# aayush9400/3D-Condtional-Stable-Diffusion

Measured on AMD Instinct MI355X. Metric: latent volumes/sec at 32^3x8ch T=1000 DDPM, higher is better.
Workload: dtype f32 (f16 hi+lo x3 MFMA, f32 accumulate)

## Files before the change

### 3d-condtional-stable-diffusion_amd/csrc/dm3d_conv.hip

```cpp
#include <algorithm>
#include <cstdlib>
#include "dm3d_conv_args.h"
#include <math.h>

namespace {

template <int TD, int TH, int TW, int S, int KS, int WM, int WN>
__global__ __launch_bounds__(256, 2) void conv3d_igemm_f32(const ConvArgs p) {
    constexpr int CK = 16, LDV = CK + 4, NT = 64;
    constexpr int TM = TD * TH * TW;
    constexpr int HD = (TD - 1) * S + KS, HH = (TH - 1) * S + KS, HW = (TW - 1) * S + KS;
    constexpr int HVOX = HD * HH * HW;
    constexpr int TAPS = KS * KS * KS;
    constexpr int MR = TM / WM / 32, NR = NT / WN / 32;
    constexpr int NTHR = WM * WN * 64;
    constexpr int NSLOT = (HVOX * 4 + NTHR - 1) / NTHR;
    static_assert(NTHR == 256, "kernel assumes 4 waves");
    static_assert(TM % (WM * 32) == 0 && NT % (WN * 32) == 0, "tile split");

    extern __shared__ __attribute__((aligned(16))) float smem[];
    float* lds_in = smem;
    float* lds_w = smem + HVOX * LDV;

    const int tid = threadIdx.x;
// ... 127 lines not shown
        const int n = n0 + wn * (NT / WN) + nr * 32 + l32;
        const bool n_ok = n < p.cout;
        const int nc = n_ok ? n : p.cout - 1;
        float add = p.bias ? p.bias[nc] : 0.0f;
        if (p.vec) add += p.vec[(size_t)vrow * p.vec_ld + nc];
#pragma unroll
        for (int mr = 0; mr < MR; ++mr) {
            size_t o[16];
            bool ok[16];
            float rv[16];
#pragma unroll
            for (int r = 0; r < 16; ++r) {
                const int row = wm * (TM / WM) + mr * 32 + dm3d_acc_row(r, half);
                const int oz = oz0 + row / (TH * TW), oy = oy0 + (row / TW) % TH, ox = ox0 + row % TW;
                ok[r] = n_ok && oz < p.od && oy < p.oh && ox < p.ow;
                o[r] = ok[r] ? ((((size_t)b * p.fd + oz * p.os + ooz) * p.fh + oy * p.os + ooy) * p.fw + ox * p.os + oox) * p.cout + n : 0;
            }
            if (p.res) {
#pragma unroll
                for (int r = 0; r < 16; ++r) rv[r] = p.res[o[r]];
            }
#pragma unroll
            for (int r = 0; r < 16; ++r) {
                float v = acc[mr][nr][r] + add;
                if (p.relu) v = fmaxf(v, 0.0f);
                if (p.prelu) { const float al = p.prelu[o[r] % sample_elems]; v = v > 0.0f ? v : al * v; }
                if (p.res) v += rv[r];
                if (p.relu_out) v = fmaxf(v, 0.0f);
                if (ok[r]) p.out[o[r]] = v;
            }
        }
    }
}

template <int TD, int TH, int TW, int S, int KS, int WM, int WN>
int launch_conv(ConvArgs& a, hipStream_t st) {
    constexpr int LDV = 20;
    constexpr int HVOX = ((TD - 1) * S + KS) * ((TH - 1) * S + KS) * ((TW - 1) * S + KS);
    constexpr size_t lds = (size_t)(HVOX * LDV + 2 * 64 * LDV) * sizeof(float);
    a.bd = (a.od + TD - 1) / TD;
    a.bh = (a.oh + TH - 1) / TH;
    a.bw = (a.ow + TW - 1) / TW;
    static std::atomic<bool> attr_set[64] = {};
    if (int dev = dm3d_dyn_lds(lds, attr_set, "conv", &conv3d_igemm_f32<TD, TH, TW, S, KS, WM, WN>); dev < 0) return dev;
    dim3 grid((unsigned)(a.batch * a.bd * a.bh * a.bw), (unsigned)(a.coutpad / 64), a.parity ? 8u : 1u);
    hipLaunchKernelGGL((conv3d_igemm_f32<TD, TH, TW, S, KS, WM, WN>), grid, dim3(256), lds, st, a);
    return dm3d_launch_check("conv3d_igemm_f32");
}

}


struct ConvKnobs {
    bool pair_off; int ksplit_mode; long split_wgs, split_target; int split_minchunks, split_maxparts; bool wino_split_off;
    int v3_td; long wide_wgs; bool wino_off; int wino_minchunks;
};
static ConvKnobs conv_knobs() {
    auto num = [](const char* name, long dflt) { const char* e = getenv(name); return e ? atol(e) : dflt; };
    auto zero = [](const char* name) { const char* e = getenv(name); return e && e[0] == '0'; };
    static const ConvKnobs once = {
        zero("DM3D_CONV_PAIR"),
        (int)num("DM3D_CONV_KSPLIT", -1),
        num("DM3D_CONV_SPLIT_WGS", 256),
        num("DM3D_CONV_SPLIT_TARGET", 512),
        (int)num("DM3D_CONV_SPLIT_MINCHUNKS", 2),
        (int)num("DM3D_CONV_SPLIT_MAXPARTS", 16),
        zero("DM3D_CONV_WINO_SPLIT"),
        0, 0, false, 0};
    ConvKnobs k = once;
    k.v3_td = (int)num("DM3D_CONV_V3_TD", 0);
    k.wide_wgs = num("DM3D_CONV_WIDE_WGS", 512);
    k.wino_off = zero("DM3D_CONV_WINO");
    k.wino_minchunks = (int)num("DM3D_CONV_WINO_MINCHUNKS", 2);
    return k;
}

static long split_tiles(const ConvArgs& a, int td) {
    return (long)a.batch * ((a.od + td - 1) / td) * ((a.oh + 7) / 8) * ((a.ow + 7) / 8) * (a.coutpad / 64) * (a.parity ? 8 : 1);
}

static int direct_ksplit(const ConvArgs& a, const ConvKnobs& K) {
    const long wgs = split_tiles(a, 4);
    if (K.ksplit_mode == 0 || wgs > K.split_wgs || a.nchunks < 4) return 1;
    int best = 1;
    for (int d = 2; d <= K.split_maxparts; ++d) {
        if (a.nchunks % d != 0 || a.nchunks / d < K.split_minchunks) continue;
        best = d;
        if (wgs * d >= K.split_target) break;
    }
    return best;
}

static int winograd_ksplit(const ConvArgs& a, const ConvKnobs& K) {
    if (K.wino_split_off || a.nchunks % 2 != 0 || a.nchunks < 16) return 1;
    const long wgs = (long)a.batch * (a.od / 8) * (a.oh / 8) * (a.ow / 8) * (a.coutpad / 64);
    return wgs <= 128 ? 2 : 1;
}

static bool winograd_serves(const ConvArgs& a, int which, int ksplit, const ConvKnobs& K) {
    if (!a.wpk_wino || which != DM3D_CONV_K3S1 || a.parity || a.cout <= 32) return false;
    if (a.s_npairs > 0) {
        if (!a.swpk_f) return false;
        const long long svox = (long long)a.batch * a.ind * a.inh * a.inw;
        if (svox * (a.sc1 > a.sc2 ? a.sc1 : a.sc2) * 4 >= (1ll << 32)) return false;
    }
    if (a.od % 8 != 0 || a.oh % 8 != 0 || a.ow % 8 != 0 || a.padz != 1 || a.pady != 1 || a.padx != 1) return false;
    if (K.wino_off || a.nchunks < K.wino_minchunks) return false;
    const long long vox = (long long)a.batch * a.ind * a.inh * a.inw;
    if (vox * (a.c1 > a.c2 ? a.c1 : a.c2) * 4 >= (1ll << 32)) return false;
    const long wgs = (long)a.batch * (a.od / 8) * (a.oh / 8) * (a.ow / 8) * (a.coutpad / 64) * ksplit;
    const long need = K.wide_wgs;
    return wgs >= need || wgs == 256 || (ksplit > 1 && wgs >= (need < 256 ? need : 256L));
}

static int direct_td(const ConvArgs& a, const ConvKnobs& K) {
    if (K.v3_td == 4) return 4;
    if (K.v3_td != 8 && (a.parity || a.s_npairs > 0)) return 4;
    if ((a.out_h2 || a.post_scale) && a.od % 8 != 0) return 4;
    return split_tiles(a, 8) >= K.wide_wgs ? 8 : 4;
}

ConvLaunch dm3d_conv_resolve(const dm3d_conv_desc* d) {
    ConvLaunch r{};
    if (!d) return r;
    const ConvKnobs K = conv_knobs();
    ConvArgs a{};
    a.x1 = d->x1; a.x2 = d->x2; a.c1 = d->c1; a.c2 = d->c2;
    a.ind = d->in_d; a.inh = d->in_h; a.inw = d->in_w;
    const bool par_mode = d->upsample || d->transpose;
    const int cstride = (par_mode || d->stride != 2) ? 1 : 2;
    a.lgd = d->in_d; a.lgh = d->in_h; a.lgw = d->in_w;
    a.od = (d->in_d + cstride - 1) / cstride;
    a.oh = (d->in_h + cstride - 1) / cstride;
    a.ow = (d->in_w + cstride - 1) / cstride;
    a.parity = par_mode ? 1 : 0;
    a.os = par_mode ? 2 : 1;
    a.fd = a.od * a.os; a.fh = a.oh * a.os; a.fw = a.ow * a.os;
    auto pad_front = [&](int in, int out) { int t = (out - 1) * cstride + d->ksize - in; return t > 0 ? t / 2 : 0; };
    a.padz = pad_front(a.lgd, a.od); a.pady = pad_front(a.lgh, a.oh); a.padx = pad_front(a.lgw, a.ow);
    const int cin = d->c1 + d->c2;
    a.cinpad = (int)dm3d_round_up(cin, DM3D_CIN_PAD);
    a.coutpad = (int)dm3d_round_up(d->cout, DM3D_COUT_PAD);
    a.nchunks = a.cinpad / 16;
    a.wpk = d->wpk; a.bias = d->bias; a.pscale = d->pro_scale; a.pshift = d->pro_shift; a.pro_bstride = d->pro_batch_stride;
    a.vec = d->vec; a.vec_idx = d->vec_idx; a.vec_ld = d->vec_ld;
    a.relu = d->relu; a.res = d->res; a.out = d->out; a.cout = d->cout;
    a.prelu = d->prelu_alpha; a.relu_out = d->relu_out;
    a.scratch = d->scratch; a.scratch_bytes = d->scratch_bytes;
    a.split_counters = d->split_counters; a.split_counter_words = d->split_counter_words;
    a.range_flag = d->range_flag; a.range_limit = d->range_limit > 0.0f ? d->range_limit : 65504.0f;
    a.wpk_wino = d->wpk_wino;
    a.x_h2 = d->x1_fmt == DM3D_FMT_H2; a.out_h2 = d->out_fmt == DM3D_FMT_H2;
    a.post_scale = d->post_scale; a.post_shift = d->post_shift;
    if (d->skip_wpk) {
        a.sx1 = d->skip_x1; a.sx2 = d->skip_x2; a.sc1 = d->skip_c1; a.sc2 = d->skip_c2; a.swpk = d->skip_wpk;
        a.s_npairs = (int)(dm3d_round_up(d->skip_c1 + d->skip_c2, 32) / 32);
        a.swpk_f = d->skip_wpk_frag;
    }
    a.batch = d->batch;
    a.out_scale = d->precision == DM3D_PREC_H3 ? ldexpf(1.0f, -d->w_exp) : 1.0f;
    if (par_mode) a.w_parity_stride = d->precision == DM3D_PREC_H3
        ? dm3d_packed_weight_h3_bytes(8, cin, d->cout) / 2 : dm3d_packed_weight_elems(8, cin, d->cout);
    a.gn_stats = d->gn_stats;
    r.a = a;
    r.which = par_mode ? DM3D_CONV_UP
                       : (d->ksize == 1 ? DM3D_CONV_K1 : (d->ksize == 4 ? DM3D_CONV_K4S2 : (d->stride == 2 ? DM3D_CONV_K3S2 : DM3D_CONV_K3S1)));

    if (d->precision != DM3D_PREC_H3) { r.family = DM3D_CONV_FAM_F32; return r; }
    if (dm3d_conv_weight_layout(d->ksize, d->stride, d->upsample, d->transpose, d->cout) != DM3D_WL_PAIR) { r.family = DM3D_CONV_FAM_TAP; return r; }
    const bool wino_geometry = r.which == DM3D_CONV_K3S1 && a.cout > 32 && a.od % 8 == 0 && a.oh % 8 == 0 && a.ow % 8 == 0;
    const int ks_direct = direct_ksplit(a, K), ks_wino = wino_geometry ? winograd_ksplit(a, K) : 1;
    auto bytes = [&](int td, int ks) { return split_tiles(a, td) * ks * (int64_t)(td * 8 * 8 * 64) * (int64_t)sizeof(float); };
    if (winograd_serves(a, r.which, a.split_counters ? ks_wino : 1, K)) {
        r.family = DM3D_CONV_FAM_WINO; r.td = 8; r.nct = 4;
        r.ksplit = a.split_counters ? ks_wino : 1;
    } else {
        r.family = DM3D_CONV_FAM_V3;
        r.nct = (r.which == DM3D_CONV_K3S1 && a.cout <= 32) ? (a.cout <= 16 ? 1 : 2) : 4;
        r.td = r.nct != 4 ? 4 : direct_td(a, K);
        r.ksplit = (r.td == 4 && a.split_counters) ? ks_direct : 1;
    }
    r.tiles = split_tiles(a, r.td);
    r.tile_floats = (long)r.td * 8 * 8 * 64;
    if (r.ksplit > 1) { r.need_words = r.tiles; r.need_bytes = bytes(r.td, r.ksplit); }
    if (d->batch <= 0 || d->cout <= 0 || d->in_d <= 0 || d->in_h <= 0 || d->in_w <= 0) return r;
    if (ks_direct > 1) { r.can_words = split_tiles(a, 4); r.can_bytes = bytes(4, ks_direct); }
    if (ks_wino > 1) { r.can_words = std::max(r.can_words, split_tiles(a, 8)); r.can_bytes = std::max(r.can_bytes, bytes(8, ks_wino)); }
    return r;
}

static int conv_validate(const dm3d_conv_desc* d) {
    DM3D_REQUIRE(d != nullptr, "conv: null descriptor");
    DM3D_REQUIRE(d->x1 && d->wpk && d->out, "conv: x1/wpk/out must be non-null");
    DM3D_REQUIRE(d->ksize == 1 || d->ksize == 3 || (d->ksize == 4 && d->stride == 2), "conv: ksize %d not in {1,3} (4 needs stride 2)", d->ksize);
    DM3D_REQUIRE(d->stride == 1 || d->stride == 2, "conv: stride %d not in {1,2}", d->stride);
    DM3D_REQUIRE(!d->transpose || (d->ksize == 4 && d->stride == 2 && !d->upsample), "conv: transpose needs ksize 4, stride 2, no upsample");
    DM3D_REQUIRE(!(d->upsample && d->stride != 1), "conv: upsample requires stride 1");
    DM3D_REQUIRE(!(d->ksize == 1 && (d->stride != 1 || d->upsample)), "conv: ksize 1 supports stride 1 without upsample only");
    DM3D_REQUIRE(d->batch > 0 && d->in_d > 0 && d->in_h > 0 && d->in_w > 0 && d->cout > 0, "conv: non-positive extent");
    DM3D_REQUIRE(d->c1 > 0 && d->c1 % 4 == 0 && d->c2 >= 0 && d->c2 % 4 == 0, "conv: c1=%d c2=%d must be multiples of 4", d->c1, d->c2);
    DM3D_REQUIRE((d->c2 == 0) == (d->x2 == nullptr), "conv: x2 and c2 must be given together");
    DM3D_REQUIRE(d->c2 == 0 || d->c1 % 16 == 0, "conv: with a second input c1=%d must be a multiple of 16", d->c1);
    DM3D_REQUIRE((d->pro_scale == nullptr) == (d->pro_shift == nullptr), "conv: pro_scale and pro_shift go together");
    DM3D_REQUIRE(!d->vec || d->vec_ld >= d->cout, "conv: vec_ld %d < cout %d", d->vec_ld, d->cout);
    const void* ptrs[] = {d->x1, d->x2, d->wpk, d->pro_scale, d->pro_shift, d->out, d->res};
    for (const void* q : ptrs) DM3D_REQUIRE(dm3d_aligned16(q), "conv: pointer %p is not 16-byte aligned", q);
    const int64_t vox = (int64_t)d->batch * d->in_d * d->in_h * d->in_w;
    DM3D_REQUIRE(vox < (1ll << 31) / 4, "conv: %lld voxels overflow the 32-bit voxel index", (long long)vox);
    DM3D_REQUIRE(d->pro_batch_stride == 0 || (d->pro_batch_stride >= d->c1 + d->c2 && d->pro_batch_stride % 4 == 0),
                 "conv: pro_batch_stride must be 0 or a multiple of 4 >= c1+c2");
    DM3D_REQUIRE((d->split_counters == nullptr) == (d->split_counter_words == 0) && d->split_counter_words >= 0, "conv: split_counters and split_counter_words go together");
    if (d->wpk_wino)
        DM3D_REQUIRE(d->precision == DM3D_PREC_H3 && dm3d_aligned16(d->wpk_wino), "conv: wpk_wino needs precision H3 and 16-byte alignment");
    DM3D_REQUIRE((d->x1_fmt == DM3D_FMT_F32 || d->x1_fmt == DM3D_FMT_H2) && (d->out_fmt == DM3D_FMT_F32 || d->out_fmt == DM3D_FMT_H2),
                 "conv: unknown x1_fmt / out_fmt");
    DM3D_REQUIRE((d->post_scale == nullptr) == (d->post_shift == nullptr), "conv: post_scale and post_shift go together");
    if (d->x1_fmt == DM3D_FMT_H2 || d->out_fmt == DM3D_FMT_H2 || d->post_scale) {
        DM3D_REQUIRE(d->precision == DM3D_PREC_H3 && d->ksize == 3 && d->stride == 1 && !d->upsample && !d->transpose,
                     "conv: x1_fmt / out_fmt / post_* need precision H3, ksize 3, stride 1, no upsample / transpose");
        DM3D_REQUIRE(d->cout > 32 || (d->out_fmt == DM3D_FMT_F32 && !d->post_scale), "conv: out_fmt H2 / post_* need cout > 32");
        DM3D_REQUIRE(d->x1_fmt != DM3D_FMT_H2 || (d->c2 == 0 && d->c1 % 16 == 0 && !d->pro_scale),
                     "conv: an H2 input needs c1 %% 16 == 0, no second input and no prologue");
        DM3D_REQUIRE(d->out_fmt != DM3D_FMT_H2 || (d->in_d % 4 == 0 && d->in_h % 8 == 0 && d->in_w % 8 == 0 && d->cout % 64 == 0 &&
                                                  !d->prelu_alpha),
                     "conv: an H2 output needs extents of whole 4x8x8 bricks and cout %% 64 == 0");
        DM3D_REQUIRE(!d->post_scale || (d->in_d % 4 == 0 && d->in_h % 8 == 0 && d->in_w % 8 == 0 && d->cout % 64 == 0),
                     "conv: post_scale needs extents of whole 4x8x8 bricks and cout %% 64 == 0");
        DM3D_REQUIRE(dm3d_aligned16(d->post_scale) && dm3d_aligned16(d->post_shift), "conv: post_* must be 16-byte aligned");
    }
    if (d->skip_wpk) {
        DM3D_REQUIRE(d->precision == DM3D_PREC_H3 && d->ksize == 3 && d->stride == 1 && !d->upsample && !d->transpose && d->cout > 32,
                     "conv: the fused skip conv needs precision H3, ksize 3, stride 1, no upsample / transpose, cout > 32");
        DM3D_REQUIRE(d->skip_x1 && d->skip_c1 > 0 && d->skip_c1 % 4 == 0 && d->skip_c2 >= 0 && d->skip_c2 % 4 == 0, "conv: skip_c1=%d skip_c2=%d must be multiples of 4", d->skip_c1, d->skip_c2);
        DM3D_REQUIRE((d->skip_c2 == 0) == (d->skip_x2 == nullptr) && (d->skip_c2 == 0 || d->skip_c1 % 16 == 0), "conv: skip_x2 / skip_c2 go together and need skip_c1 %% 16 == 0");
        DM3D_REQUIRE(dm3d_aligned16(d->skip_x1) && dm3d_aligned16(d->skip_x2) && dm3d_aligned16(d->skip_wpk), "conv: skip pointers must be 16-byte aligned");
        DM3D_REQUIRE(dm3d_aligned16(d->skip_wpk_frag), "conv: skip_wpk_frag must be 16-byte aligned");
    }
    DM3D_REQUIRE(dm3d_aligned16(d->scratch) && d->scratch_bytes >= 0, "conv: scratch must be 16-byte aligned");
    DM3D_REQUIRE(d->precision == DM3D_PREC_F32 || d->precision == DM3D_PREC_H3, "conv: unknown precision %d", d->precision);
    DM3D_REQUIRE(d->w_exp >= -100 && d->w_exp <= 100, "conv: w_exp %d out of range", d->w_exp);
    if (d->gn_stats)
        DM3D_REQUIRE(d->out_fmt == DM3D_FMT_F32 && d->cout % 4 == 0 && dm3d_aligned16(d->gn_stats),
                     "conv: gn_stats needs a float32 output, cout %% 4 == 0 and a 16-byte aligned buffer");
    if (d->precision == DM3D_PREC_H3) {
        const int layout = dm3d_conv_weight_layout(d->ksize, d->stride, d->upsample, d->transpose, d->cout);
        DM3D_REQUIRE(d->w_layout == layout, "conv: w_layout %d but this geometry reads layout %d (dm3d_conv_weight_layout)", d->w_layout, layout);
    }
    return DM3D_OK;
}

extern "C" int dm3d_conv3d_ndhwc(const dm3d_conv_desc* d, void* stream) {
    if (int rc = conv_validate(d)) return rc;
    ConvLaunch r = dm3d_conv_resolve(d);
    hipStream_t st = static_cast<hipStream_t>(stream);
    if (r.family == DM3D_CONV_FAM_WINO) return dm3d_conv_launch_h3w(r, st);
    if (r.family == DM3D_CONV_FAM_V3) return dm3d_conv_launch_h3v3(r, st);
    const int rc = r.family == DM3D_CONV_FAM_TAP ? dm3d_conv_launch_h3(r.a, r.which, st) : dm3d_conv_launch_f32(r.a, r.which, st);
    if (rc != DM3D_OK || !r.a.gn_stats) return rc;
    return dm3d_groupnorm_partials(r.a.out, r.a.batch, (int64_t)r.a.fd * r.a.fh * r.a.fw, r.a.cout, r.a.gn_stats, stream);
}

extern "C" int64_t dm3d_packed_weight_skip_h3p_bytes(int32_t cin, int32_t cout) {
    return (cin > 0 && cout > 0) ? dm3d_h3v2_skip_image_bytes(cin, cout) : 0;
}

extern "C" int dm3d_pack_weights_skip_h3p(const float* keras_kernel, int32_t cin, int32_t cout, int32_t w_exp, void* packed, void* stream) {
    DM3D_REQUIRE(keras_kernel && packed && cin > 0 && cout > 0, "pack_weights_skip_h3p: bad arguments");
    DM3D_REQUIRE(w_exp >= -100 && w_exp <= 100 && dm3d_aligned16(packed), "pack_weights_skip_h3p: w_exp out of range or packed unaligned");
    return dm3d_pack_skip_h3v2(keras_kernel, cin, cout, w_exp, packed, static_cast<hipStream_t>(stream));
}

extern "C" int dm3d_pack_weights_skip_h3f(const float* keras_kernel, int32_t cin, int32_t cout, int32_t w_exp, void* packed, void* stream) {
    DM3D_REQUIRE(keras_kernel && packed && cin > 0 && cout > 0, "pack_weights_skip_h3f: bad arguments");
    DM3D_REQUIRE(w_exp >= -100 && w_exp <= 100 && dm3d_aligned16(packed), "pack_weights_skip_h3f: w_exp out of range or packed unaligned");
    return dm3d_pack_skip_h3f(keras_kernel, cin, cout, w_exp, packed, static_cast<hipStream_t>(stream));
}

extern "C" int32_t dm3d_conv_tile_form(const dm3d_conv_desc* d) {
    const ConvLaunch r = dm3d_conv_resolve(d);
    return r.family == DM3D_CONV_FAM_WINO ? 10 : (r.family == DM3D_CONV_FAM_V3 ? r.td : 0);
}

extern "C" int64_t dm3d_conv_scratch_bytes(const dm3d_conv_desc* d) { return dm3d_conv_resolve(d).can_bytes; }

extern "C" int32_t dm3d_conv_split_counter_words(const dm3d_conv_desc* d) { return (int32_t)dm3d_conv_resolve(d).can_words; }

extern "C" int32_t dm3d_conv_weight_layout(int32_t ksize, int32_t stride, int32_t upsample, int32_t transpose, int32_t cout) {
    (void)cout;
    if (conv_knobs().pair_off) return DM3D_WL_TAP;
    if (upsample || transpose) return DM3D_WL_PAIR;
    return (ksize == 3 && stride == 1) ? DM3D_WL_PAIR : DM3D_WL_TAP;
}

extern "C" int64_t dm3d_packed_weight_h3p_bytes(int32_t taps, int32_t cin, int32_t cout) {
    if (taps <= 0 || cin <= 0 || cout <= 0) return 0;
    return dm3d_h3v2_image_bytes(taps, cin, cout);
}

extern "C" int dm3d_pack_weights_h3p(const float* keras_kernel, int32_t taps, int32_t cin, int32_t cout, int32_t w_exp,
                                     const float* in_scale, void* packed, int32_t mode, void* stream) {
    DM3D_REQUIRE(keras_kernel && packed && taps > 0 && cin > 0 && cout > 0, "pack_weights_h3p: bad arguments");
    DM3D_REQUIRE(mode >= 0 && mode <= 2 && (mode == 0 || taps == 8), "pack_weights_h3p: mode %d with taps %d", mode, taps);
    DM3D_REQUIRE(w_exp >= -100 && w_exp <= 100, "pack_weights_h3p: w_exp %d out of range", w_exp);
    DM3D_REQUIRE(dm3d_aligned16(packed), "pack_weights_h3p: packed must be 16-byte aligned");
    return dm3d_pack_h3v2(keras_kernel, taps, cin, cout, w_exp, in_scale, packed, mode, static_cast<hipStream_t>(stream));
}

extern "C" int64_t dm3d_packed_weight_h3w_bytes(int32_t cin, int32_t cout) {
    if (cin <= 0 || cout <= 0) return 0;
    return dm3d_h3v2_image_bytes(40, cin, cout);
// ... 18 lines not shown
```

### 3d-condtional-stable-diffusion_amd/csrc/dm3d_conv_args.h

```cpp
#pragma once
#include "dm3d_common.h"

struct ConvArgs {
    const float* x1; const float* x2; int c1, c2;
    int ind, inh, inw;
    int lgd, lgh, lgw;
    int od, oh, ow;
    int padz, pady, padx;
    int os;
    int ooz, ooy, oox;
    int fd, fh, fw;
    int parity;
    long w_parity_stride;
    const void* wpk; int cinpad, coutpad;
    const float* bias; const float* pscale; const float* pshift; long pro_bstride;
    const float* vec; const int* vec_idx; int vec_ld;
    int relu; const float* res; float* out; int cout;
    const float* prelu; int relu_out;
    int bd, bh, bw;
    int nchunks;
    int batch;
    float out_scale;
    int ksplit;
    int* split_counters;
    int split_counter_words;
    long split_tile_floats;
    void* scratch; long scratch_bytes;
    const float* post_scale; const float* post_shift;
    int out_h2;
    int x_h2;
    const float* sx1; const float* sx2; int sc1, sc2; const void* swpk; int s_npairs;
    const void* swpk_f;
    const void* wpk_wino;
    int* range_flag; float range_limit;
    float* gn_stats;
    int epi_vec4;
};

enum { DM3D_CONV_K3S1 = 0, DM3D_CONV_K3S2 = 1, DM3D_CONV_K1 = 2, DM3D_CONV_UP = 3, DM3D_CONV_K4S2 = 4 };

enum { DM3D_CONV_FAM_F32 = 0,
       DM3D_CONV_FAM_TAP = 1,
       DM3D_CONV_FAM_V3 = 2,
       DM3D_CONV_FAM_WINO = 3 };

struct ConvLaunch {
    ConvArgs a;
    int which;
    int family;
    int td;
    int nct;
    int ksplit;
    long tiles, tile_floats;
    int64_t need_bytes; long need_words;
    int64_t can_bytes; long can_words;
};
ConvLaunch dm3d_conv_resolve(const dm3d_conv_desc* d);

int dm3d_conv_launch_f32(ConvArgs& a, int which, hipStream_t st);
int dm3d_conv_launch_h3(ConvArgs& a, int which, hipStream_t st);
int dm3d_conv_launch_h3v3(const ConvLaunch& r, hipStream_t st);
int dm3d_conv_launch_h3w(const ConvLaunch& r, hipStream_t st);
struct H3v2Launch { ConvArgs k; bool stats_after; };
int dm3d_h3v2_pre_launch(const ConvLaunch& r, H3v2Launch& L);
int dm3d_h3v2_post_launch(const ConvArgs& a, const H3v2Launch& L, hipStream_t st);
int64_t dm3d_h3v2_skip_image_bytes(int cin, int cout);
int dm3d_pack_skip_h3v2(const float* keras_kernel, int cin, int cout, int w_exp, void* packed, hipStream_t st);
int dm3d_pack_skip_h3f(const float* keras_kernel, int cin, int cout, int w_exp, void* packed, hipStream_t st);
int64_t dm3d_h3v2_image_bytes(int taps, int cin, int cout);
int dm3d_pack_h3v2(const float* keras_kernel, int taps, int cin, int cout, int w_exp, const float* in_scale, void* packed, int mode,
                   hipStream_t st);
```

### 3d-condtional-stable-diffusion_amd/csrc/dm3d_conv_h3.hip

```cpp
#include "dm3d_conv_args.h"
#include "dm3d_h3.h"

namespace {

constexpr int REC = DM3D_REC;

template <int PAIR>
__device__ __forceinline__ void row_to_yx(int i, int& dy, int& dx) {
    if (PAIR == 0) { dy = i >> 3; dx = i & 7; return; }
    const bool g1 = (i >= 4 && i < 12) || (i >= 16 && i < 20) || i >= 28;
    const int idx = g1 ? (i < 12 ? i - 4 : (i < 20 ? i - 8 : i - 16)) : (i < 4 ? i : (i < 16 ? i - 8 : i - 12));
    const int sel = idx >> 3;
    dx = idx & 7;
    if (PAIR == 2) dy = g1 ? 1 + 2 * sel : 2 * sel;
    else dy = g1 ? 2 + sel : sel;
}

template <int TD, int TH, int TW, int S, int KS, int WM, int WN, int MINW, int NRA = 0>
__global__ __launch_bounds__(256, MINW) void conv3d_igemm_h3(const ConvArgs p) {
    constexpr int CK = 16, NT = 64;
    constexpr int TM = TD * TH * TW;
    constexpr int HD = (TD - 1) * S + KS, HH = (TH - 1) * S + KS, HW = (TW - 1) * S + KS;
    constexpr int HVOX = HD * HH * HW;
    constexpr bool CF = (S == 1 && TH % 4 == 0 && TW == 8);
    constexpr int HWP = (CF && KS >= 2) ? 12 : HW;
    constexpr int PAIR = CF ? (KS >= 2 ? 2 : 1) : 0;
    constexpr int HREC = HD * HH * HWP;
    constexpr int MRSTEP = 4 * S * HWP;
    static_assert(TM / WM <= 32 || MRSTEP % 16 == 0, "row tiles of a wave must share the swizzle term");
    static_assert(TM / WM <= TH * TW, "a wave's rows stay inside one z slice");
    constexpr int TAPS = KS * KS * KS;
    constexpr int G = KS;
    constexpr int NG = TAPS / G;
    constexpr int MR = TM / WM / 32, NR = NRA > 0 ? NRA : NT / WN / 32;
    constexpr int NSLOT = (HVOX * 2 + 255) / 256;
    constexpr int WGRP = G * NT * REC;
    constexpr int WPIECES = WGRP * 2 / 16;
    constexpr int WSLOT = WPIECES / 256;
    static_assert(WPIECES % 256 == 0, "a weight group is a whole number of 16-byte pieces per thread (no guards: a guarded "
                                      "load costs a serialized vmcnt(0))");
    static_assert(WM * WN == 4, "kernel assumes 4 waves");
    static_assert(TW == 8 && (TM / WM) % 32 == 0 && (TH * TW) % 32 == 0, "a 32-row MFMA tile is 4 x 8 voxels of one z");

    extern __shared__ __attribute__((aligned(16))) _Float16 smem_h[];
    _Float16* lds_in = smem_h;
    _Float16* lds_w = smem_h + HREC * REC;

    const int tid = threadIdx.x;
    const int lane = tid & 63, wave = tid >> 6;
    const int half = lane >> 5, l32 = lane & 31;
    const int wm = wave / WN, wn = wave % WN;

    int brick = blockIdx.x;
    const int bpv = p.bd * p.bh * p.bw;
    const int b = brick / bpv;
    brick -= b * bpv;
    const int oz0 = (brick / (p.bh * p.bw)) * TD;
    const int oy0 = ((brick / p.bw) % p.bh) * TH;
    const int ox0 = (brick % p.bw) * TW;
    const int ntile = blockIdx.y;
    int padz = p.padz, pady = p.pady, padx = p.padx, ooz = p.ooz, ooy = p.ooy, oox = p.oox;
    const _Float16* wbase = static_cast<const _Float16*>(p.wpk);
    if (p.parity) {
        const int par = blockIdx.z;
        ooz = par >> 2; ooy = (par >> 1) & 1; oox = par & 1;
        padz = 1 - ooz; pady = 1 - ooy; padx = 1 - oox;
        wbase += (size_t)par * p.w_parity_stride;
    }

// ... 130 lines not shown
            const int kd = g / KS, kh = g % KS;
            const _Float16* wbuf = lds_w + (g & 1) * WGRP;
#pragma unroll
            for (int t = 0; t < G; ++t) {
                const int tap_rec = (kd * HH + kh) * HWP + t;
                h8 ah[MR], al[MR], bh[NR], bl[NR];
                {
                    const int v = a_rec[0] + tap_rec;
                    const int hi_off = v * REC + ((half ^ swz(v)) << 3);
                    const int lo_off = hi_off ^ 16;
#pragma unroll
                    for (int mr = 0; mr < MR; ++mr) {
                        ah[mr] = *reinterpret_cast<const h8*>(lds_in + hi_off + mr * (MRSTEP * REC));
                        al[mr] = *reinterpret_cast<const h8*>(lds_in + lo_off + mr * (MRSTEP * REC));
                    }
                }
#pragma unroll
                for (int nr = 0; nr < NR; ++nr) {
                    bh[nr] = *reinterpret_cast<const h8*>(wbuf + t * (NT * REC) + b_hi[nr]);
                    bl[nr] = *reinterpret_cast<const h8*>(wbuf + t * (NT * REC) + b_lo[nr]);
                }
#ifndef DM3D_MFMA_PASS_MAJOR
#pragma unroll
                for (int mr = 0; mr < MR; ++mr)
#pragma unroll
                    for (int nr = 0; nr < NR; ++nr) {
                        acc[mr][nr] = __builtin_amdgcn_mfma_f32_32x32x16_f16(al[mr], bh[nr], acc[mr][nr], 0, 0, 0);
                        acc[mr][nr] = __builtin_amdgcn_mfma_f32_32x32x16_f16(ah[mr], bl[nr], acc[mr][nr], 0, 0, 0);
                        acc[mr][nr] = __builtin_amdgcn_mfma_f32_32x32x16_f16(ah[mr], bh[nr], acc[mr][nr], 0, 0, 0);
                    }
#else
#pragma unroll
                for (int mr = 0; mr < MR; ++mr)
#pragma unroll
                    for (int nr = 0; nr < NR; ++nr) acc[mr][nr] = __builtin_amdgcn_mfma_f32_32x32x16_f16(al[mr], bh[nr], acc[mr][nr], 0, 0, 0);
#pragma unroll
                for (int mr = 0; mr < MR; ++mr)
#pragma unroll
                    for (int nr = 0; nr < NR; ++nr) acc[mr][nr] = __builtin_amdgcn_mfma_f32_32x32x16_f16(ah[mr], bl[nr], acc[mr][nr], 0, 0, 0);
#pragma unroll
                for (int mr = 0; mr < MR; ++mr)
#pragma unroll
                    for (int nr = 0; nr < NR; ++nr) acc[mr][nr] = __builtin_amdgcn_mfma_f32_32x32x16_f16(ah[mr], bh[nr], acc[mr][nr], 0, 0, 0);
#endif
            }
            __builtin_amdgcn_sched_barrier(0);
            if (!last_group) {
                store_w((g + 1) & 1);
                __syncthreads();
            }
        }
    }

    const int vrow = p.vec ? (p.vec_idx ? p.vec_idx[b] : b) : 0;
    const int n0 = ntile * NT;
    const bool full = oz0 + TD <= p.od && oy0 + TH <= p.oh && ox0 + TW <= p.ow && n0 + NT <= p.cout;
    const int cstep = p.os * p.cout;
    float amax = 0.0f;
#pragma unroll
    for (int mr = 0; mr < MR; ++mr) {
        const int r0 = wm * (TM / WM) + mr * 32;
        const int oz = oz0 + r0 / (TH * TW), oyb = oy0 + (r0 / TW) % TH;
        const bool z_ok = oz < p.od;
        const size_t zbase = (((size_t)b * p.fd + (z_ok ? oz * p.os + ooz : 0)) * p.fh) * p.fw * p.cout;
        float* outz = p.out + zbase;
        const float* resz = p.res ? p.res + zbase : nullptr;
        const float* prz = p.prelu ? p.prelu + (zbase - (size_t)b * p.fd * p.fh * p.fw * p.cout) : nullptr;
        int rowoff[4], oyq[4], oxq[4];
#pragma unroll
        for (int q = 0; q < 4; ++q) {
            int dy, dx;
            row_to_yx<PAIR>(8 * q + 4 * half, dy, dx);
            oyq[q] = oyb + dy;
            oxq[q] = ox0 + dx;
            rowoff[q] = ((oyq[q] * p.os + ooy) * p.fw + oxq[q] * p.os + oox) * p.cout;
        }
#pragma unroll
        for (int nr = 0; nr < NR; ++nr) {
            const int n = n0 + wn * (NT / WN) + nr * 32 + l32;
            const bool n_ok = n < p.cout;
            const int nc = n_ok ? n : p.cout - 1;
            float add = p.bias ? p.bias[nc] : 0.0f;
            if (p.vec) add += p.vec[(size_t)vrow * p.vec_ld + nc];
            if (full) {
                float rv[16];
                if (resz) {
#pragma unroll
                    for (int r = 0; r < 16; ++r) rv[r] = resz[rowoff[r >> 2] + (r & 3) * cstep + n];
                }
#pragma unroll
                for (int r = 0; r < 16; ++r) {
                    const int o = rowoff[r >> 2] + (r & 3) * cstep + n;
                    float v = fmaf(acc[mr][nr][r], p.out_scale, add);
                    if (p.relu) v = fmaxf(v, 0.0f);
                    if (prz) { const float al = prz[o]; v = v > 0.0f ? v : al * v; }
                    if (resz) v += rv[r];
                    if (p.relu_out) v = fmaxf(v, 0.0f);
                    DM3D_AMAX(amax, v);
                    outz[o] = v;
                }
            } else {
#pragma unroll
                for (int r = 0; r < 16; ++r) {
                    const int q = r >> 2, c = r & 3;
                    const bool ok = n_ok && z_ok && oyq[q] < p.oh && oxq[q] + c < p.ow;
                    const int o = ok ? rowoff[q] + c * cstep + n : 0;
                    float v = fmaf(acc[mr][nr][r], p.out_scale, add);
                    if (p.relu) v = fmaxf(v, 0.0f);
                    if (prz) { const float al = prz[o]; v = v > 0.0f ? v : al * v; }
                    if (resz) v += resz[o];
                    if (p.relu_out) v = fmaxf(v, 0.0f);
                    if (ok) { DM3D_AMAX(amax, v); outz[o] = v; }
                }
            }
        }
    }
    if (p.range_flag && amax > p.range_limit) *p.range_flag = 1;
}

template <int TD, int TH, int TW, int S, int KS, int WM, int WN, int MINW, int NRA = 0>
int launch_h3(ConvArgs& a, hipStream_t st) {
    constexpr int HW = (TW - 1) * S + KS;
    constexpr int HWP = (S == 1 && TH % 4 == 0 && TW == 8 && KS >= 2) ? 12 : HW;
    constexpr int HREC = ((TD - 1) * S + KS) * ((TH - 1) * S + KS) * HWP;
    constexpr size_t lds = (size_t)(HREC * REC + 2 * KS * 64 * REC) * sizeof(_Float16);
    static_assert(lds <= 160 * 1024, "LDS budget");
    a.bd = (a.od + TD - 1) / TD;
    a.bh = (a.oh + TH - 1) / TH;
    a.bw = (a.ow + TW - 1) / TW;
    static std::atomic<bool> attr_set[64] = {};
    if (int dev = dm3d_dyn_lds(lds, attr_set, "conv", &conv3d_igemm_h3<TD, TH, TW, S, KS, WM, WN, MINW, NRA>); dev < 0) return dev;
    dim3 grid((unsigned)(a.batch * a.bd * a.bh * a.bw), (unsigned)(a.coutpad / 64), a.parity ? 8u : 1u);
    hipLaunchKernelGGL((conv3d_igemm_h3<TD, TH, TW, S, KS, WM, WN, MINW, NRA>), grid, dim3(256), lds, st, a);
    return dm3d_launch_check("conv3d_igemm_h3");
}

__global__ __launch_bounds__(256) void pack_weights_h3_kernel(const float* __restrict__ w, int taps, int cin, int cout,
                                                              int nchunks, int ntiles, float scale, const float* in_scale,
                                                              _Float16* __restrict__ out, int up) {
    const long nrec = (long)ntiles * nchunks * taps * 64;
    for (long i0 = (long)blockIdx.x * 256 + threadIdx.x; i0 < nrec * 16 * (up ? 8 : 1); i0 += (long)gridDim.x * 256) {
        const int par = (int)(i0 / (nrec * 16));
        const long i = i0 % (nrec * 16);
        const int k = (int)(i & 15);
        long rec = i >> 4;
        const int nn = (int)(rec % 64);
        const int tap = (int)((rec / 64) % taps);
        const int chunk = (int)((rec / (64L * taps)) % nchunks);
        const int nt = (int)(rec / (64L * taps * nchunks));
        const int ci = chunk * 16 + k, co = nt * 64 + nn;
        float v = 0.f;
        if (ci < cin && co < cout) {
            v = up == 1 ? dm3d_up_weight(w, cin, cout, par, tap, ci, co)
              : up == 2 ? dm3d_convt_weight(w, cin, cout, par, tap, ci, co) : w[((long)tap * cin + ci) * cout + co];
            if (in_scale) v *= in_scale[ci];
            v *= scale;
        }
        const _Float16 hi = (_Float16)v;
        const _Float16 lo = (_Float16)(v - (float)hi);
        _Float16* r = out + ((long)par * nrec + rec) * REC;
        const int sw = (nn >> 2) & 3;
        r[(((k >> 3) ^ sw) << 3) + (k & 7)] = hi;
        r[(((2 + (k >> 3)) ^ sw) << 3) + (k & 7)] = lo;
    }
}

}

int dm3d_conv_launch_h3(ConvArgs& a, int which, hipStream_t st) {
    if (which == DM3D_CONV_UP) return launch_h3<4, 8, 8, 1, 2, 4, 1, 2>(a, st);
// ... 52 lines not shown
```

Before: 2.195.

## Add dedicated stride-2 3x3x3 h3 conv kernel with parity-split halo and weight ring

Adds a specialized kernel for the stride-2 k3 convolutions that previously went through the generic tap kernel. It stores the input halo in LDS split by x parity so strided taps read contiguous records. It streams weights through a three-slot register/LDS ring, overlapping the next halo load and conversion with the MFMA work. Tile depth (2 or 4) is picked from the workgroup count to keep the GPU occupied, and the shared epilogue is moved into a header. The cost is extra code paths, and occupancy is limited to one workgroup per CU by the launch bounds.

```diff
diff --git a/3d-condtional-stable-diffusion_amd/csrc/dm3d_conv.hip b/3d-condtional-stable-diffusion_amd/csrc/dm3d_conv.hip
--- a/3d-condtional-stable-diffusion_amd/csrc/dm3d_conv.hip
+++ b/3d-condtional-stable-diffusion_amd/csrc/dm3d_conv.hip
@@ -203,8 +203,8 @@
 
 
 struct ConvKnobs {
-    bool pair_off; int ksplit_mode; long split_wgs, split_target; int split_minchunks, split_maxparts; bool wino_split_off;
-    int v3_td; long wide_wgs; bool wino_off; int wino_minchunks;
+    bool pair_off; int ksplit_mode; long split_wgs, split_target; int split_minchunks, split_maxparts; bool wino_split_off; bool s2_legacy;
+    int s2_td; int v3_td; long wide_wgs; bool wino_off; int wino_minchunks;
 };
 static ConvKnobs conv_knobs() {
     auto num = [](const char* name, long dflt) { const char* e = getenv(name); return e ? atol(e) : dflt; };
@@ -217,8 +217,10 @@
         (int)num("DM3D_CONV_SPLIT_MINCHUNKS", 2),
         (int)num("DM3D_CONV_SPLIT_MAXPARTS", 16),
         zero("DM3D_CONV_WINO_SPLIT"),
-        0, 0, false, 0};
+        num("DM3D_CONV_S2_LEGACY", 0) == 1,
+        0, 0, 0, false, 0};
     ConvKnobs k = once;
+    k.s2_td = (int)num("DM3D_CONV_S2_TD", 0);
     k.v3_td = (int)num("DM3D_CONV_V3_TD", 0);
     k.wide_wgs = num("DM3D_CONV_WIDE_WGS", 512);
     k.wino_off = zero("DM3D_CONV_WINO");
@@ -269,6 +271,12 @@
     if (K.v3_td != 8 && (a.parity || a.s_npairs > 0)) return 4;
     if ((a.out_h2 || a.post_scale) && a.od % 8 != 0) return 4;
     return split_tiles(a, 8) >= K.wide_wgs ? 8 : 4;
+}
+
+static int s2_depth(const ConvArgs& a, const ConvKnobs& K) {
+    if (K.s2_td == 2 || K.s2_td == 4) return K.s2_td;
+    const long wgs = (long)a.batch * ((a.od + 3) / 4) * ((a.oh + 3) / 4) * ((a.ow + 7) / 8) * (a.coutpad / 64);
+    return 2 * wgs <= 256 ? 2 : 4;
 }
 
 ConvLaunch dm3d_conv_resolve(const dm3d_conv_desc* d) {
@@ -318,7 +326,11 @@
                        : (d->ksize == 1 ? DM3D_CONV_K1 : (d->ksize == 4 ? DM3D_CONV_K4S2 : (d->stride == 2 ? DM3D_CONV_K3S2 : DM3D_CONV_K3S1)));
 
     if (d->precision != DM3D_PREC_H3) { r.family = DM3D_CONV_FAM_F32; return r; }
-    if (dm3d_conv_weight_layout(d->ksize, d->stride, d->upsample, d->transpose, d->cout) != DM3D_WL_PAIR) { r.family = DM3D_CONV_FAM_TAP; return r; }
+    if (dm3d_conv_weight_layout(d->ksize, d->stride, d->upsample, d->transpose, d->cout) != DM3D_WL_PAIR) {
+        r.family = DM3D_CONV_FAM_TAP;
+        if (r.which == DM3D_CONV_K3S2 && !K.s2_legacy) r.s2_td = s2_depth(a, K);
+        return r;
+    }
     const bool wino_geometry = r.which == DM3D_CONV_K3S1 && a.cout > 32 && a.od % 8 == 0 && a.oh % 8 == 0 && a.ow % 8 == 0;
     const int ks_direct = direct_ksplit(a, K), ks_wino = wino_geometry ? winograd_ksplit(a, K) : 1;
     auto bytes = [&](int td, int ks) { return split_tiles(a, td) * ks * (int64_t)(td * 8 * 8 * 64) * (int64_t)sizeof(float); };
@@ -406,7 +418,8 @@
     hipStream_t st = static_cast<hipStream_t>(stream);
     if (r.family == DM3D_CONV_FAM_WINO) return dm3d_conv_launch_h3w(r, st);
     if (r.family == DM3D_CONV_FAM_V3) return dm3d_conv_launch_h3v3(r, st);
-    const int rc = r.family == DM3D_CONV_FAM_TAP ? dm3d_conv_launch_h3(r.a, r.which, st) : dm3d_conv_launch_f32(r.a, r.which, st);
+    const int rc = r.family != DM3D_CONV_FAM_TAP ? dm3d_conv_launch_f32(r.a, r.which, st)
+                 : (r.s2_td ? dm3d_conv_launch_h3s2(r.a, r.s2_td, st) : dm3d_conv_launch_h3(r.a, r.which, st));
     if (rc != DM3D_OK || !r.a.gn_stats) return rc;
     return dm3d_groupnorm_partials(r.a.out, r.a.batch, (int64_t)r.a.fd * r.a.fh * r.a.fw, r.a.cout, r.a.gn_stats, stream);
 }
diff --git a/3d-condtional-stable-diffusion_amd/csrc/dm3d_conv_args.h b/3d-condtional-stable-diffusion_amd/csrc/dm3d_conv_args.h
--- a/3d-condtional-stable-diffusion_amd/csrc/dm3d_conv_args.h
+++ b/3d-condtional-stable-diffusion_amd/csrc/dm3d_conv_args.h
@@ -51,6 +51,7 @@
     int td;
     int nct;
     int ksplit;
+    int s2_td;
     long tiles, tile_floats;
     int64_t need_bytes; long need_words;
     int64_t can_bytes; long can_words;
@@ -59,6 +60,7 @@
 
 int dm3d_conv_launch_f32(ConvArgs& a, int which, hipStream_t st);
 int dm3d_conv_launch_h3(ConvArgs& a, int which, hipStream_t st);
+int dm3d_conv_launch_h3s2(ConvArgs& a, int td, hipStream_t st);
 int dm3d_conv_launch_h3v3(const ConvLaunch& r, hipStream_t st);
 int dm3d_conv_launch_h3w(const ConvLaunch& r, hipStream_t st);
 struct H3v2Launch { ConvArgs k; bool stats_after; };
diff --git a/3d-condtional-stable-diffusion_amd/csrc/dm3d_conv_h3.hip b/3d-condtional-stable-diffusion_amd/csrc/dm3d_conv_h3.hip
--- a/3d-condtional-stable-diffusion_amd/csrc/dm3d_conv_h3.hip
+++ b/3d-condtional-stable-diffusion_amd/csrc/dm3d_conv_h3.hip
@@ -1,20 +1,10 @@
 #include "dm3d_conv_args.h"
 #include "dm3d_h3.h"
+#include "dm3d_conv_h3_parts.h"
 
 namespace {
 
 constexpr int REC = DM3D_REC;
-
-template <int PAIR>
-__device__ __forceinline__ void row_to_yx(int i, int& dy, int& dx) {
-    if (PAIR == 0) { dy = i >> 3; dx = i & 7; return; }
-    const bool g1 = (i >= 4 && i < 12) || (i >= 16 && i < 20) || i >= 28;
-    const int idx = g1 ? (i < 12 ? i - 4 : (i < 20 ? i - 8 : i - 16)) : (i < 4 ? i : (i < 16 ? i - 8 : i - 12));
-    const int sel = idx >> 3;
-    dx = idx & 7;
-    if (PAIR == 2) dy = g1 ? 1 + 2 * sel : 2 * sel;
-    else dy = g1 ? 2 + sel : sel;
-}
 
 template <int TD, int TH, int TW, int S, int KS, int WM, int WN, int MINW, int NRA = 0>
 __global__ __launch_bounds__(256, MINW) void conv3d_igemm_h3(const ConvArgs p) {
@@ -251,70 +241,7 @@
         }
     }
 
-    const int vrow = p.vec ? (p.vec_idx ? p.vec_idx[b] : b) : 0;
-    const int n0 = ntile * NT;
-    const bool full = oz0 + TD <= p.od && oy0 + TH <= p.oh && ox0 + TW <= p.ow && n0 + NT <= p.cout;
-    const int cstep = p.os * p.cout;
-    float amax = 0.0f;
-#pragma unroll
-    for (int mr = 0; mr < MR; ++mr) {
-        const int r0 = wm * (TM / WM) + mr * 32;
-        const int oz = oz0 + r0 / (TH * TW), oyb = oy0 + (r0 / TW) % TH;
-        const bool z_ok = oz < p.od;
-        const size_t zbase = (((size_t)b * p.fd + (z_ok ? oz * p.os + ooz : 0)) * p.fh) * p.fw * p.cout;
-        float* outz = p.out + zbase;
-        const float* resz = p.res ? p.res + zbase : nullptr;
-        const float* prz = p.prelu ? p.prelu + (zbase - (size_t)b * p.fd * p.fh * p.fw * p.cout) : nullptr;
-        int rowoff[4], oyq[4], oxq[4];
-#pragma unroll
-        for (int q = 0; q < 4; ++q) {
-            int dy, dx;
-            row_to_yx<PAIR>(8 * q + 4 * half, dy, dx);
-            oyq[q] = oyb + dy;
-            oxq[q] = ox0 + dx;
-            rowoff[q] = ((oyq[q] * p.os + ooy) * p.fw + oxq[q] * p.os + oox) * p.cout;
-        }
-#pragma unroll
-        for (int nr = 0; nr < NR; ++nr) {
-            const int n = n0 + wn * (NT / WN) + nr * 32 + l32;
-            const bool n_ok = n < p.cout;
-            const int nc = n_ok ? n : p.cout - 1;
-            float add = p.bias ? p.bias[nc] : 0.0f;
-            if (p.vec) add += p.vec[(size_t)vrow * p.vec_ld + nc];
-            if (full) {
-                float rv[16];
-                if (resz) {
-#pragma unroll
-                    for (int r = 0; r < 16; ++r) rv[r] = resz[rowoff[r >> 2] + (r & 3) * cstep + n];
-                }
-#pragma unroll
-                for (int r = 0; r < 16; ++r) {
-                    const int o = rowoff[r >> 2] + (r & 3) * cstep + n;
-                    float v = fmaf(acc[mr][nr][r], p.out_scale, add);
-                    if (p.relu) v = fmaxf(v, 0.0f);
-                    if (prz) { const float al = prz[o]; v = v > 0.0f ? v : al * v; }
-                    if (resz) v += rv[r];
-                    if (p.relu_out) v = fmaxf(v, 0.0f);
-                    DM3D_AMAX(amax, v);
-                    outz[o] = v;
-                }
-            } else {
-#pragma unroll
-                for (int r = 0; r < 16; ++r) {
-                    const int q = r >> 2, c = r & 3;
-                    const bool ok = n_ok && z_ok && oyq[q] < p.oh && oxq[q] + c < p.ow;
-                    const int o = ok ? rowoff[q] + c * cstep + n : 0;
-                    float v = fmaf(acc[mr][nr][r], p.out_scale, add);
-                    if (p.relu) v = fmaxf(v, 0.0f);
-                    if (prz) { const float al = prz[o]; v = v > 0.0f ? v : al * v; }
-                    if (resz) v += resz[o];
-                    if (p.relu_out) v = fmaxf(v, 0.0f);
-                    if (ok) { DM3D_AMAX(amax, v); outz[o] = v; }
-                }
-            }
-        }
-    }
-    if (p.range_flag && amax > p.range_limit) *p.range_flag = 1;
+    h3_tap_epilogue<PAIR, TD, TH, TW, WM, WN, MR, NR>(p, acc, b, oz0, oy0, ox0, ooz, ooy, oox, ntile, wm, wn, half, l32);
 }
 
 template <int TD, int TH, int TW, int S, int KS, int WM, int WN, int MINW, int NRA = 0>
diff --git a/3d-condtional-stable-diffusion_amd/csrc/dm3d_conv_h3_parts.h b/3d-condtional-stable-diffusion_amd/csrc/dm3d_conv_h3_parts.h
--- /dev/null
+++ b/3d-condtional-stable-diffusion_amd/csrc/dm3d_conv_h3_parts.h
@@ -0,0 +1,84 @@
+#pragma once
+#include "dm3d_conv_args.h"
+#include "dm3d_h3.h"
+
+template <int PAIR>
+__device__ __forceinline__ void row_to_yx(int i, int& dy, int& dx) {
+    if (PAIR == 0) { dy = i >> 3; dx = i & 7; return; }
+    const bool g1 = (i >= 4 && i < 12) || (i >= 16 && i < 20) || i >= 28;
+    const int idx = g1 ? (i < 12 ? i - 4 : (i < 20 ? i - 8 : i - 16)) : (i < 4 ? i : (i < 16 ? i - 8 : i - 12));
+    const int sel = idx >> 3;
+    dx = idx & 7;
+    if (PAIR == 2) dy = g1 ? 1 + 2 * sel : 2 * sel;
+    else dy = g1 ? 2 + sel : sel;
+}
+
+template <int PAIR, int TD, int TH, int TW, int WM, int WN, int MR, int NR>
+__device__ __forceinline__ void h3_tap_epilogue(const ConvArgs& p, const f32x16 (&acc)[MR][NR], int b, int oz0, int oy0, int ox0, int ooz, int ooy,
+                                                int oox, int ntile, int wm, int wn, int half, int l32) {
+    constexpr int NT = 64, TM = TD * TH * TW;
+    const int vrow = p.vec ? (p.vec_idx ? p.vec_idx[b] : b) : 0;
+    const int n0 = ntile * NT;
+    const bool full = oz0 + TD <= p.od && oy0 + TH <= p.oh && ox0 + TW <= p.ow && n0 + NT <= p.cout;
+    const int cstep = p.os * p.cout;
+    float amax = 0.0f;
+#pragma unroll
+    for (int mr = 0; mr < MR; ++mr) {
+        const int r0 = wm * (TM / WM) + mr * 32;
+        const int oz = oz0 + r0 / (TH * TW), oyb = oy0 + (r0 / TW) % TH;
+        const bool z_ok = oz < p.od;
+        const size_t zbase = (((size_t)b * p.fd + (z_ok ? oz * p.os + ooz : 0)) * p.fh) * p.fw * p.cout;
+        float* outz = p.out + zbase;
+        const float* resz = p.res ? p.res + zbase : nullptr;
+        const float* prz = p.prelu ? p.prelu + (zbase - (size_t)b * p.fd * p.fh * p.fw * p.cout) : nullptr;
+        int rowoff[4], oyq[4], oxq[4];
+#pragma unroll
+        for (int q = 0; q < 4; ++q) {
+            int dy, dx;
+            row_to_yx<PAIR>(8 * q + 4 * half, dy, dx);
+            oyq[q] = oyb + dy;
+            oxq[q] = ox0 + dx;
+            rowoff[q] = ((oyq[q] * p.os + ooy) * p.fw + oxq[q] * p.os + oox) * p.cout;
+        }
+#pragma unroll
+        for (int nr = 0; nr < NR; ++nr) {
+            const int n = n0 + wn * (NT / WN) + nr * 32 + l32;
+            const bool n_ok = n < p.cout;
+            const int nc = n_ok ? n : p.cout - 1;
+            float add = p.bias ? p.bias[nc] : 0.0f;
+            if (p.vec) add += p.vec[(size_t)vrow * p.vec_ld + nc];
+            if (full) {
+                float rv[16];
+                if (resz) {
+#pragma unroll
+                    for (int r = 0; r < 16; ++r) rv[r] = resz[rowoff[r >> 2] + (r & 3) * cstep + n];
+                }
+#pragma unroll
+                for (int r = 0; r < 16; ++r) {
+                    const int o = rowoff[r >> 2] + (r & 3) * cstep + n;
+                    float v = fmaf(acc[mr][nr][r], p.out_scale, add);
+                    if (p.relu) v = fmaxf(v, 0.0f);
+                    if (prz) { const float al = prz[o]; v = v > 0.0f ? v : al * v; }
+                    if (resz) v += rv[r];
+                    if (p.relu_out) v = fmaxf(v, 0.0f);
+                    DM3D_AMAX(amax, v);
+                    outz[o] = v;
+                }
+            } else {
+#pragma unroll
+                for (int r = 0; r < 16; ++r) {
+                    const int q = r >> 2, c = r & 3;
+                    const bool ok = n_ok && z_ok && oyq[q] < p.oh && oxq[q] + c < p.ow;
+                    const int o = ok ? rowoff[q] + c * cstep + n : 0;
+                    float v = fmaf(acc[mr][nr][r], p.out_scale, add);
+                    if (p.relu) v = fmaxf(v, 0.0f);
+                    if (prz) { const float al = prz[o]; v = v > 0.0f ? v : al * v; }
+                    if (resz) v += resz[o];
+                    if (p.relu_out) v = fmaxf(v, 0.0f);
+                    if (ok) { DM3D_AMAX(amax, v); outz[o] = v; }
+                }
+            }
+        }
+    }
+    if (p.range_flag && amax > p.range_limit) *p.range_flag = 1;
+}
diff --git a/3d-condtional-stable-diffusion_amd/csrc/dm3d_conv_h3s2.hip b/3d-condtional-stable-diffusion_amd/csrc/dm3d_conv_h3s2.hip
--- /dev/null
+++ b/3d-condtional-stable-diffusion_amd/csrc/dm3d_conv_h3s2.hip
@@ -0,0 +1,233 @@
+#include "dm3d_conv_h3_parts.h"
+
+namespace {
+
+constexpr int REC = DM3D_REC;
+
+template <int TD, int WM, int WN>
+__global__ __launch_bounds__(256, 1) void conv3d_s2_h3(const ConvArgs p) {
+    constexpr int TH = 4, TW = 8, CK = 16, NT = 64;
+    constexpr int TM = TD * TH * TW;
+    constexpr int HD = 2 * TD + 1, HH = 2 * TH + 1, HW = 2 * TW + 1;
+    constexpr int XODD = TW + 1;
+    constexpr int HWP = 18;
+    constexpr int HVOX = HD * HH * HW, HREC = HD * HH * HWP;
+    constexpr int NG = 9, G = 3, RING = 3;
+    constexpr int MR = TM / WM / 32, NR = NT / WN / 32;
+    constexpr int NSLOT = (HVOX * 2 + 255) / 256;
+    constexpr int WGRP = G * NT * REC, WPIECES = WGRP * 2 / 16, WSLOT = WPIECES / 256;
+    constexpr int CV0 = 3, CVN = (NSLOT + NG - CV0 - 1) / (NG - CV0);
+    static_assert(WM * WN == 4 && MR == 1 && TM / WM == TH * TW, "four waves, one 32-row tile (one z slice) each");
+    static_assert(NG % RING == 0 && WPIECES % 256 == 0, "ring slots are compile-time; whole 16-byte pieces per thread");
+
+    extern __shared__ __attribute__((aligned(16))) _Float16 smem_s2[];
+    _Float16* lds_in = smem_s2;
+    _Float16* lds_w = smem_s2 + HREC * REC;
+
+    const int tid = threadIdx.x;
+    const int lane = tid & 63, wave = tid >> 6;
+    const int half = lane >> 5, l32 = lane & 31;
+    const int wm = wave / WN, wn = wave % WN;
+
+    int brick = blockIdx.x;
+    const int bpv = p.bd * p.bh * p.bw;
+    const int b = brick / bpv;
+    brick -= b * bpv;
+    const int oz0 = (brick / (p.bh * p.bw)) * TD;
+    const int oy0 = ((brick / p.bw) % p.bh) * TH;
+    const int ox0 = (brick % p.bw) * TW;
+    const int ntile = blockIdx.y;
+
+    const int piece = tid & 1;
+    int gvox[NSLOT], st_off[NSLOT];
+#pragma unroll
+    for (int j = 0; j < NSLOT; ++j) {
+        const int hv = (tid >> 1) + j * 128;
+        int g = -1, so = -1;
+        if (hv < HVOX) {
+            const int hz = hv / (HH * HW), hy = (hv / HW) % HH, hx = hv % HW;
+            const int iz = oz0 * 2 - p.padz + hz, iy = oy0 * 2 - p.pady + hy, ix = ox0 * 2 - p.padx + hx;
+            if (iz >= 0 && iz < p.ind && iy >= 0 && iy < p.inh && ix >= 0 && ix < p.inw)
+                g = ((b * p.ind + iz) * p.inh + iy) * p.inw + ix;
+            const int v = (hz * HH + hy) * HWP + (hx & 1) * XODD + (hx >> 1);
+            so = v * REC + ((piece ^ swz(v)) << 3);
+        }
+        gvox[j] = g;
+        st_off[j] = so;
+    }
+
+    int a_rec;
+    {
+        int dy, dx;
+        row_to_yx<2>(l32, dy, dx);
+        a_rec = (wm * 2 * HH + dy * 2) * HWP + dx;
+    }
+    int b_hi[NR], b_lo[NR];
+#pragma unroll
+    for (int nr = 0; nr < NR; ++nr) {
+        const int n = wn * (NT / WN) + nr * 32 + l32;
+        b_hi[nr] = n * REC + ((half ^ swz(n)) << 3);
+        b_lo[nr] = n * REC + (((2 + half) ^ swz(n)) << 3);
+    }
+
+    f32x16 acc[MR][NR];
+#pragma unroll
+    for (int nr = 0; nr < NR; ++nr)
+#pragma unroll
+        for (int r = 0; r < 16; ++r) acc[0][nr][r] = 0.0f;
+
+    const f32x4* w_img = reinterpret_cast<const f32x4*>(static_cast<const _Float16*>(p.wpk) + (size_t)ntile * p.nchunks * NG * WGRP);
+    const int lastg = p.nchunks * NG - 1;
+    f32x4 wreg[RING][WSLOT];
+    auto fetch_w = [&](int gi, const int set) {
+        const f32x4* src = w_img + (size_t)(gi < lastg ? gi : lastg) * WPIECES;
+#pragma unroll
+        for (int i = 0; i < WSLOT; ++i) wreg[set][i] = src[tid + i * 256];
+    };
+    auto store_w = [&](const int set, const int buf) {
+        f32x4* dst = reinterpret_cast<f32x4*>(lds_w + buf * WGRP);
+#pragma unroll
+        for (int i = 0; i < WSLOT; ++i) dst[tid + i * 256] = wreg[set][i];
+    };
+    auto lds_barrier = [&]() {
+        asm volatile("s_waitcnt lgkmcnt(0)" ::: "memory");
+        __builtin_amdgcn_s_barrier();
+        asm volatile("" ::: "memory");
+    };
+
+    const bool pro = p.pscale != nullptr;
+    f32x4 raw0[NSLOT], raw1[NSLOT];
+    f32x4 sc0 = {1.f, 1.f, 1.f, 1.f}, sc1 = sc0, sh0 = {0.f, 0.f, 0.f, 0.f}, sh1 = sh0;
+    bool ok0 = false, ok1 = false;
+    auto load_halo = [&](int ch) {
+        const int c0 = ch * CK;
+        const float* src;
+        int ldc, cb;
+        if (c0 < p.c1) { src = p.x1; ldc = p.c1; cb = c0; } else { src = p.x2; ldc = p.c2; cb = c0 - p.c1; }
+        const int cpos = cb + piece * 8;
+        ok0 = cpos < ldc;
+        ok1 = cpos + 4 < ldc;
+        const int off0 = ok0 ? cpos : 0, off1 = ok1 ? cpos + 4 : 0;
+#pragma unroll
+        for (int j = 0; j < NSLOT; ++j) {
+            const float* q = src + (size_t)(gvox[j] >= 0 ? gvox[j] : 0) * ldc;
+            raw0[j] = *reinterpret_cast<const f32x4*>(q + off0);
+            raw1[j] = *reinterpret_cast<const f32x4*>(q + off1);
+        }
+        if (pro) {
+            const int s0 = ok0 ? c0 + piece * 8 : 0, s1 = ok1 ? c0 + piece * 8 + 4 : 0;
+            const size_t bo = (size_t)b * p.pro_bstride;
+            sc0 = *reinterpret_cast<const f32x4*>(p.pscale + bo + s0);
+            sh0 = *reinterpret_cast<const f32x4*>(p.pshift + bo + s0);
+            sc1 = *reinterpret_cast<const f32x4*>(p.pscale + bo + s1);
+            sh1 = *reinterpret_cast<const f32x4*>(p.pshift + bo + s1);
+        }
+    };
+    auto convert_slot = [&](const int j) {
+        const bool in = gvox[j] >= 0;
+        f32x4 v0 = raw0[j], v1 = raw1[j];
+        if (pro) {
+#pragma unroll
+            for (int e = 0; e < 4; ++e) {
+                v0[e] = dm3d_silu(fmaf(v0[e], sc0[e], sh0[e]));
+                v1[e] = dm3d_silu(fmaf(v1[e], sc1[e], sh1[e]));
+            }
+        }
+        h8 hi, lo;
+        split8(v0, v1, (in && ok0) ? 65504.0f : 0.0f, (in && ok1) ? 65504.0f : 0.0f, hi, lo);
+        raw0[j] = __builtin_bit_cast(f32x4, hi);
+        raw1[j] = __builtin_bit_cast(f32x4, lo);
+    };
+    auto store_image = [&]() {
+#pragma unroll
+        for (int j = 0; j < NSLOT; ++j) {
+            if (st_off[j] >= 0) {
+                *reinterpret_cast<f32x4*>(lds_in + st_off[j]) = raw0[j];
+                *reinterpret_cast<f32x4*>(lds_in + (st_off[j] ^ 16)) = raw1[j];
+            }
+        }
+    };
+
+    struct Frag { h8 ah, al, bh[NR], bl[NR]; };
+    auto read_frag = [&](Frag& f, const int g, const int t) {
+        const int v = a_rec + ((g / 3) * HH + g % 3) * HWP + (t == 1 ? XODD : t >> 1);
+        const int hi_off = v * REC + ((half ^ swz(v)) << 3);
+        f.ah = *reinterpret_cast<const h8*>(lds_in + hi_off);
+        f.al = *reinterpret_cast<const h8*>(lds_in + (hi_off ^ 16));
+        const _Float16* wbuf = lds_w + (g % RING) * WGRP + t * (NT * REC);
+#pragma unroll
+        for (int nr = 0; nr < NR; ++nr) {
+            f.bh[nr] = *reinterpret_cast<const h8*>(wbuf + b_hi[nr]);
+            f.bl[nr] = *reinterpret_cast<const h8*>(wbuf + b_lo[nr]);
+        }
+    };
+
+    fetch_w(0, 0);
+    fetch_w(1, 1);
+    load_halo(0);
+    store_w(0, 0);
+    store_w(1, 1);
+#pragma unroll
+    for (int i = 0; i < RING; ++i) fetch_w(2 + i, i);
+#pragma unroll
+    for (int j = 0; j < NSLOT; ++j) convert_slot(j);
+    store_image();
+    lds_barrier();
+
+    Frag fr[2];
+    for (int ch = 0; ch < p.nchunks; ++ch) {
+        read_frag(fr[0], 0, 0);
+        load_halo(ch + 1 < p.nchunks ? ch + 1 : ch);
+        __builtin_amdgcn_sched_barrier(0);
+#pragma unroll
+        for (int g = 0; g < NG; ++g) {
+            store_w(g % RING, (g + 2) % RING);
+            fetch_w(ch * NG + g + 2 + RING, g % RING);
+            __builtin_amdgcn_sched_barrier(0);
+#pragma unroll
+            for (int t = 0; t < G; ++t) {
+                const int k = g * G + t;
+                Frag& cur = fr[k & 1];
+                if (k + 1 < NG * G) read_frag(fr[(k + 1) & 1], (k + 1) / G, (k + 1) % G);
+                __builtin_amdgcn_sched_barrier(0);
+#pragma unroll
+                for (int nr = 0; nr < NR; ++nr) acc[0][nr] = __builtin_amdgcn_mfma_f32_32x32x16_f16(cur.al, cur.bh[nr], acc[0][nr], 0, 0, 0);
+#pragma unroll
+                for (int nr = 0; nr < NR; ++nr) acc[0][nr] = __builtin_amdgcn_mfma_f32_32x32x16_f16(cur.ah, cur.bl[nr], acc[0][nr], 0, 0, 0);
+#pragma unroll
+                for (int nr = 0; nr < NR; ++nr) acc[0][nr] = __builtin_amdgcn_mfma_f32_32x32x16_f16(cur.ah, cur.bh[nr], acc[0][nr], 0, 0, 0);
+                if (t == 0 && g >= CV0) {
+#pragma unroll
+                    for (int j = (g - CV0) * CVN; j < (g - CV0 + 1) * CVN && j < NSLOT; ++j) convert_slot(j);
+                }
+                __builtin_amdgcn_sched_barrier(0);
+            }
+            lds_barrier();
+        }
+        store_image();
+        lds_barrier();
+    }
+
+    h3_tap_epilogue<2, TD, TH, TW, WM, WN, MR, NR>(p, acc, b, oz0, oy0, ox0, p.ooz, p.ooy, p.oox, ntile, wm, wn, half, l32);
+}
+
+template <int TD, int WM, int WN>
+int launch_s2(ConvArgs& a, hipStream_t st) {
+    constexpr int HREC = (2 * TD + 1) * 9 * 18;
+    constexpr size_t lds = (size_t)(HREC * REC + 3 * 3 * 64 * REC) * sizeof(_Float16);
+    static_assert(lds <= 160 * 1024, "LDS budget");
+    a.bd = (a.od + TD - 1) / TD;
+    a.bh = (a.oh + 3) / 4;
+    a.bw = (a.ow + 7) / 8;
+    static std::atomic<bool> attr_set[64] = {};
+    if (int dev = dm3d_dyn_lds(lds, attr_set, "conv", &conv3d_s2_h3<TD, WM, WN>); dev < 0) return dev;
+    dim3 grid((unsigned)(a.batch * a.bd * a.bh * a.bw), (unsigned)(a.coutpad / 64), 1u);
+    hipLaunchKernelGGL((conv3d_s2_h3<TD, WM, WN>), grid, dim3(256), lds, st, a);
+    return dm3d_launch_check("conv3d_s2_h3");
+}
+
+}
+
+int dm3d_conv_launch_h3s2(ConvArgs& a, int td, hipStream_t st) {
+    return td == 2 ? launch_s2<2, 2, 2>(a, st) : launch_s2<4, 4, 1>(a, st);
+}
```

Measured after the change: 2.194 (median of 2 runs). No clear change (-0.1%).
